# santurini/vsrlab

Measured on AMD Instinct MI355X. Metric: LR frames/sec fwd+bwd, BasicVSR 4x 540p 7-frame clip, 1->8 MI355X, higher is better.
Workload: dtype bf16; 1 GPU; BasicVSR(mid=64,res_blocks=30,x4) fwd+Charbonnier+bwd+clip+Adam, 540x960->2160x3840, 7-frame clip, 2 clips per GPU (BASELINE configs[1]); clips_per_gpu=2, frames=7, res_blocks=30, parallelism=single GPU, arena=full, train_flow=False, trunk_chains=True

## Files before the change

vsrlab_amd/csrc/conv3x3_c64_tile.h:

```cpp
#pragma once
#include "common.h"

constexpr int PTW = 32, PTH = 8, PNT = 512;
constexpr int PTWH = PTW + 2, PTHH = PTH + 2, PNPIX = PTHH * PTWH;
constexpr int W_BYTES = 9 * 64 * 64 * 2;
constexpr int IN_BYTES = PNPIX * 128;
constexpr int BIAS_OFF = W_BYTES + 2 * IN_BYTES;
constexpr int IN_CHUNKS = PNPIX * 8;
constexpr int NPIECE_T = (IN_CHUNKS + 63) / 64;
constexpr int NPIECE_W = (NPIECE_T + 3) / 4;
constexpr int WCH = 9 * 64 * 8 / 256;

typedef __attribute__((ext_vector_type(2))) __bf16 bf16x2_t;
typedef __attribute__((ext_vector_type(4))) unsigned u32x4_t;
typedef __attribute__((ext_vector_type(2))) unsigned u32x2_t;
#define GP(T, x) ((__attribute__((address_space(1))) T*)(x))

static __device__ __forceinline__ unsigned pk_bf16(float a, float b) {
    bf16x2_t p = {(bf16_t)a, (bf16_t)b};
    return __builtin_bit_cast(unsigned, p);
}
static __device__ __forceinline__ unsigned pk_max_i16(unsigned a, unsigned b) { unsigned r; asm("v_pk_max_i16 %0, %1, %2" : "=v"(r) : "v"(a), "v"(b)); return r; }
static __device__ __forceinline__ unsigned pk_min_u16(unsigned a, unsigned b) { unsigned r; asm("v_pk_min_u16 %0, %1, %2" : "=v"(r) : "v"(a), "v"(b)); return r; }
static __device__ __forceinline__ unsigned pk_mul_lo_u16(unsigned a, unsigned b) { unsigned r; asm("v_pk_mul_lo_u16 %0, %1, %2" : "=v"(r) : "v"(a), "v"(b)); return r; }
// ... 54 lines not shown
#define C64_RES_IDENTITY(idA, l15, q)                                                                                    \
    bf16x8_t idA[2];                                                                                                     \
    _Pragma("unroll") for (int hb = 0; hb < 2; ++hb)                                                                     \
        _Pragma("unroll") for (int j = 0; j < 8; ++j) idA[hb][j] = (bf16_t)(((q) == ((l15) >> 2) && j == 4 * hb + ((l15) & 3)) ? 1.f : 0.f);
#define C64_ADD_RESIDUAL(acc, idA, rr)                                                                                 \
    _Pragma("unroll") for (int nb = 0; nb < 4; ++nb)                                                                   \
        _Pragma("unroll") for (int mb = 0; mb < 4; ++mb)                                                               \
            acc[mb][nb] = __builtin_amdgcn_mfma_f32_16x16x32_bf16(idA[mb & 1], __builtin_bit_cast(bf16x8_t, rr[mb >> 1][nb]), acc[mb][nb], 0, 0, 0);

#define C64_DSR(dst, addr, imm) asm volatile("ds_read_b128 %0, %1 offset:%2" : "=v"(dst) : "v"(addr), "i"(imm))
#define C64_LOADA(tap_, kk_, slot, mb)                                                                                 \
    C64_DSR(fa_[slot][mb], (tap_ < 6 ? a_lo[kk_] : a_hi[kk_]), (tap_ < 6 ? tap_ : tap_ - 6) * 8192 + (mb) * 2048);
#define C64_LOADB(ky_, kx_, kk_, slot, nb)                                                                             \
    C64_DSR(fb_[slot][nb], bb_, (((nb) >> 1) + ky_) * (PTWH * 128) + kk_ * (4 * PTWH * 16) + (((nb) & 1) * 16 + kx_) * 16);
#define C64_LOAD(s, slot)                                                                                              \
    {                                                                                                                  \
        constexpr int tap_ = (s) / 2, kk_ = (s) % 2, ky_ = tap_ / 3, kx_ = tap_ % 3;                                   \
        C64_LOADA(tap_, kk_, slot, 0) C64_LOADA(tap_, kk_, slot, 1) C64_LOADA(tap_, kk_, slot, 2) C64_LOADA(tap_, kk_, slot, 3) \
        C64_LOADB(ky_, kx_, kk_, slot, 0) C64_LOADB(ky_, kx_, kk_, slot, 1) C64_LOADB(ky_, kx_, kk_, slot, 2) C64_LOADB(ky_, kx_, kk_, slot, 3) \
    }
#define C64_MFMA(acc, bvec, s, mb, nb) acc[mb][nb] = __builtin_amdgcn_mfma_f32_16x16x32_bf16(fa_[(s) % 2][mb], fb_[(s) % 2][nb], (s) == 0 ? bvec[mb] : acc[mb][nb], 0, 0, 0);
#define C64_ML_A(acc, bvec, s, mb, nb, lmb)                                                                            \
    C64_MFMA(acc, bvec, s, mb, nb)                                                                                     \
    __builtin_amdgcn_sched_barrier(0);                       \
    if ((s) + 1 < 18) { constexpr int t1_ = ((s) + 1) / 2, k1_ = ((s) + 1) % 2; C64_LOADA(t1_, k1_, ((s) + 1) % 2, lmb) } \
    __builtin_amdgcn_sched_barrier(0);
#define C64_ML_B(acc, bvec, s, mb, nb, lnb)                                                                            \
    C64_MFMA(acc, bvec, s, mb, nb)                                                                                     \
    __builtin_amdgcn_sched_barrier(0);                                                                                 \
    if ((s) + 1 < 18) { constexpr int t1_ = ((s) + 1) / 2, k1_ = ((s) + 1) % 2; C64_LOADB(t1_ / 3, t1_ % 3, k1_, ((s) + 1) % 2, lnb) } \
    __builtin_amdgcn_sched_barrier(0);
#define C64_STEP(acc, bvec, s)                                                                                         \
    {                                                                                                                  \
        asm volatile("s_waitcnt lgkmcnt(0)" ::: "memory");                                 \
        __builtin_amdgcn_sched_barrier(0);                                                                             \
        C64_ML_A(acc, bvec, s, 0, 0, 0) C64_ML_A(acc, bvec, s, 0, 1, 1) C64_ML_A(acc, bvec, s, 0, 2, 2) C64_ML_A(acc, bvec, s, 0, 3, 3) \
        C64_ML_B(acc, bvec, s, 1, 0, 0) C64_ML_B(acc, bvec, s, 1, 1, 1) C64_ML_B(acc, bvec, s, 1, 2, 2) C64_ML_B(acc, bvec, s, 1, 3, 3) \
        C64_MFMA(acc, bvec, s, 2, 0) C64_MFMA(acc, bvec, s, 2, 1) C64_MFMA(acc, bvec, s, 2, 2) C64_MFMA(acc, bvec, s, 2, 3)  \
        C64_MFMA(acc, bvec, s, 3, 0) C64_MFMA(acc, bvec, s, 3, 1) C64_MFMA(acc, bvec, s, 3, 2) C64_MFMA(acc, bvec, s, 3, 3)  \
        __builtin_amdgcn_sched_barrier(0);                                                                             \
    }
#define C64_K_LOOP(acc, bvec, cur)                                                                                                    \
    {                                                                                                                  \
        bf16x8_t fa_[2][4], fb_[2][4];                                                                                 \
        const unsigned bb_ = (unsigned)(W_BYTES + (cur) * IN_BYTES + (b_lane));      \
        asm volatile("s_waitcnt lgkmcnt(0)" ::: "memory");                         \
        __builtin_amdgcn_sched_barrier(0);                                                                             \
        C64_LOAD(0, 0)                                                                                                 \
        C64_STEP(acc, bvec, 0) C64_STEP(acc, bvec, 1) C64_STEP(acc, bvec, 2) C64_STEP(acc, bvec, 3) C64_STEP(acc, bvec, 4) C64_STEP(acc, bvec, 5) \
        C64_STEP(acc, bvec, 6) C64_STEP(acc, bvec, 7) C64_STEP(acc, bvec, 8) C64_STEP(acc, bvec, 9) C64_STEP(acc, bvec, 10) C64_STEP(acc, bvec, 11) \
        C64_STEP(acc, bvec, 12) C64_STEP(acc, bvec, 13) C64_STEP(acc, bvec, 14) C64_STEP(acc, bvec, 15) C64_STEP(acc, bvec, 16) C64_STEP(acc, bvec, 17) \
    }

constexpr unsigned C64_K11 = 0x00010001u;
#define C64_ARM_PLAIN(ow, v)                                                                                             \
    _Pragma("unroll") for (int jj = 0; jj < 4; ++jj) ow[jj] = pk_bf16(v[2 * jj], v[2 * jj + 1]);
#define C64_ARM_RELU(ow, v, nb, sign_k)                                                                                  \
    _Pragma("unroll") for (int jj = 0; jj < 4; ++jj) {                                                                   \
        ow[jj] = pk_max_i16(pk_bf16(v[2 * jj], v[2 * jj + 1]), 0u);                                                      \
        sign_k |= pk_min_u16(ow[jj], C64_K11) << (4 * (nb) + jj);                                                        \
    }
#define C64_ARM_MASKED(ow, v, nb, wbits)                                                                                 \
    _Pragma("unroll") for (int jj = 0; jj < 4; ++jj)                                                                     \
        ow[jj] = pk_mul_lo_u16(pk_bf16(v[2 * jj], v[2 * jj + 1]), ((wbits) >> (4 * (nb) + jj)) & C64_K11);
static __device__ __forceinline__ long long c64_sign_word(int tile, int w4, int lane) { return (long long)tile * 256 + w4 * 64 + lane; }
```

vsrlab_amd/csrc/conv3x3_persist.hip:

```cpp
#include "conv3x3_c64_tile.h"
#include <type_traits>

namespace {

constexpr int P_LDS = BIAS_OFF + 256;

__device__ uint4 g_conv_zero_chunk[2];

template <int ACT> __device__ __forceinline__ float p_act(float v, float slope) {
    if (ACT == ACT_RELU) return v > 0.f ? v : 0.f;
    if (ACT == ACT_LEAKY) return v > 0.f ? v : slope * v;
    return v;
}

#ifdef VSR_CLOCK
__device__ unsigned long long g_clk[256 * 4];
#endif

__device__ __forceinline__ void tile_coords(int tile, int ntx, int nty, int& n, int& ty0, int& tx0) {
    const int per = ntx * nty;
    n = tile / per;
    const int r = tile - n * per;
    const int ty = r / ntx;
    ty0 = ty * PTH;
    tx0 = (r - ty * ntx) * PTW;
}

struct TileIter {
    int tile, n, ty, tx;
    int sn, sty, stx;
    __device__ __forceinline__ void init(int first, int stride, int ntx, int nty) {
        const int per = ntx * nty;
        tile = first; n = first / per; int r = first - n * per; ty = r / ntx; tx = r - ty * ntx;
        sn = stride / per; r = stride - sn * per; sty = r / ntx; stx = r - sty * ntx;
    }
    __device__ __forceinline__ void advance(int stride, int ntx, int nty) {
        tile += stride;
        tx += stx; if (tx >= ntx) { tx -= ntx; ++ty; }
        ty += sty; if (ty >= nty) { ty -= nty; ++n; }
        n += sn;
    }
};

__device__ __forceinline__ float bf_lo(unsigned w) { return __uint_as_float(w << 16); }
__device__ __forceinline__ float bf_hi(unsigned w) { return __uint_as_float(w & 0xffff0000u); }

constexpr int DMA_PLAIN = 0;

template <int ACT, bool HAS_RES, int MASK>
__global__ __launch_bounds__(PNT, 1) void conv3x3_c64_persist_kernel(const ConvArgs ka) {
    extern __shared__ __attribute__((aligned(16))) char smem[];

    const int z = blockIdx.y;
// ... 165 lines not shown
                                }
                            }
                            C64_ARM_PLAIN(ow, v)
                        }
                        const u32x4_t o = {ow[0], ow[1], ow[2], ow[3]};
                        *GP(u32x4_t, dst + k * 1024) = o;
                    }
                }
            }
            };
            if (full) epilogue(std::true_type{}); else epilogue(std::false_type{});
            if (ACT != ACT_NONE && !HAS_RES && sout_z) sout_z[c64_sign_word(tile, w4, lane)] = u32x2_t{sout[0], sout[1]};
            __syncthreads();
            cur ^= 1;
        }
    }
#ifdef VSR_CLOCK
    if (tid == 0 && blockIdx.y == 0 && blockIdx.x < 256) {
        g_clk[blockIdx.x * 4 + 0] = __builtin_amdgcn_s_memtime() - clk_t0;
        g_clk[blockIdx.x * 4 + 1] = __builtin_amdgcn_s_memrealtime() - clk_r0;
    }
#endif
}

__global__ void sign_bits_c64_kernel(const bf16_t* __restrict__ x, uint2* __restrict__ bits, int N, int H, int W) {
    const int ntx = cdiv(W, PTW), nty = cdiv(H, PTH);
    const long long total = (long long)N * ntx * nty * 256;
    const long long gid = (long long)blockIdx.x * blockDim.x + threadIdx.x;
    if (gid >= total) return;
    const int lane = (int)(gid & 63), w4 = (int)((gid >> 6) & 3);
    const int tile = (int)(gid >> 8);
    const int l15 = lane & 15, q = lane >> 4;
    const int pxl = PM_LANE_PIXEL(l15);
    int n, ty0, tx0;
    tile_coords(tile, ntx, nty, n, ty0, tx0);
    unsigned out[2] = {0u, 0u};
#pragma unroll
    for (int nb = 0; nb < 4; ++nb) {
        const int yy = ty0 + 2 * w4 + (nb >> 1), xx = tx0 + (nb & 1) * 16 + pxl;
        if (yy < H && xx < W) {
#pragma unroll
            for (int k = 0; k < 2; ++k) {
                const uint4 v = *reinterpret_cast<const uint4*>(x + (long long)n * pm_image_elems(H, W, 64) + pm_off(yy, xx, 4 * k + q, W, 64));
                const unsigned vw[4] = {v.x, v.y, v.z, v.w};
#pragma unroll
                for (int jj = 0; jj < 4; ++jj)
                    out[k] |= ((bf_lo(vw[jj]) > 0.f ? 1u : 0u) | (bf_hi(vw[jj]) > 0.f ? 0x10000u : 0u)) << (4 * nb + jj);
            }
        }
    }
    bits[gid] = make_uint2(out[0], out[1]);
}

template <int ACT, bool HAS_RES, int MASK>
static int launch_persist(const ConvArgs& a, int num_cus, hipStream_t st) {
    auto kern = conv3x3_c64_persist_kernel<ACT, HAS_RES, MASK>;
    static VsrDevOnce once;
    { const int rc = vsr_set_max_dynamic_lds(once, reinterpret_cast<const void*>(kern), P_LDS); if (rc != VSR_OK) return rc; }
    const int tiles = a.N * cdiv(a.W, PTW) * cdiv(a.H, PTH);
    int gx = num_cus / a.nz;
    gx &= ~7;
    if (gx < 8) gx = num_cus / a.nz;
    if (gx < 1) gx = 1;
    if (gx > tiles) gx = tiles;
    hipLaunchKernelGGL(kern, dim3(gx, a.nz), dim3(PNT), P_LDS, st, a);
    HIP_CHECK_RET(hipGetLastError());
    return VSR_OK;
}

}

#ifdef VSR_CLOCK
extern "C" int vsr_debug_read_clk(unsigned long long* host_out) {
    return hipMemcpyFromSymbol(host_out, HIP_SYMBOL(g_clk), sizeof(unsigned long long) * 256 * 4) == hipSuccess ? 0 : -3;
}
#endif

int vsr_launch_conv3x3_c64_persist(const ConvArgs& a, int num_cus, hipStream_t st) {
    bool res = false, aux = false;
    for (int z = 0; z < a.nz; ++z) { res = res || a.res[z]; aux = aux || a.aux[z]; }
    for (int z = 0; z < a.nz; ++z) if ((res && !a.res[z]) || (aux && !a.aux[z])) return VSR_ERR_UNSUPPORTED;
    int mask = aux ? a.mask_mode : MASK_NONE;
    if (mask == MASK_RELU && !res) {
        bool bits = true;
        for (int z = 0; z < a.nz; ++z) bits = bits && a.sign_bits[z];
        if (bits) mask = MASK_RELU_BITS;
    }
    if (mask == MASK_LEAKY && res) {
        bool bits = true;
        for (int z = 0; z < a.nz; ++z) bits = bits && a.sign_bits[z];
        if (bits) mask = MASK_LEAKY_BITS;
    }
    if (pm_image_elems((PTHH + 2) * a.in_step, a.Ws, 64) * 2 > 0x7fffffffLL || pm_image_elems(2 * PTH + 2, a.Wd, 64) > 0x7fffffffLL)
        return VSR_ERR_UNSUPPORTED;
    if (a.unshuffle) {
        if (a.nz != 1 || a.out_step != 1 || a.out_ox[0] || a.out_oy[0] || (a.Hd & 1) || (a.Wd & 1) || a.Hd != a.H || a.Wd != a.W || aux ||
            a.unshuffle_plane < (long long)a.N * pm_image_elems(a.Hd / 2, a.Wd / 2, 64) || a.dst_nstride != pm_image_elems(a.Hd / 2, a.Wd / 2, 64) ||
            3 * a.unshuffle_plane + pm_image_elems(PTH + 2, a.Wd / 2, 64) > 0x7fffffffLL)
            return VSR_ERR_UNSUPPORTED;
    }
#define PERSIST_CASE(ACT, RES, MASK) if (a.act == ACT && res == RES && mask == MASK) return launch_persist<ACT, RES, MASK>(a, num_cus, st);
    PERSIST_CASE(ACT_RELU, false, MASK_NONE)
    PERSIST_CASE(ACT_NONE, true, MASK_NONE)
    PERSIST_CASE(ACT_LEAKY, false, MASK_NONE)
    PERSIST_CASE(ACT_NONE, false, MASK_NONE)
    PERSIST_CASE(ACT_NONE, false, MASK_RELU)
    PERSIST_CASE(ACT_NONE, false, MASK_RELU_BITS)
    PERSIST_CASE(ACT_NONE, true, MASK_LEAKY)
    PERSIST_CASE(ACT_NONE, true, MASK_LEAKY_BITS)
    PERSIST_CASE(ACT_NONE, false, MASK_LEAKY)
#undef PERSIST_CASE
    return VSR_ERR_UNSUPPORTED;
}

int vsr_launch_sign_bits_c64(const void* x_pm, void* bits, int N, int H, int W, hipStream_t st) {
    if (!x_pm || !bits || N < 1 || H < 1 || W < 1) return VSR_ERR_BADARG;
    const long long total = (long long)N * cdiv(W, PTW) * cdiv(H, PTH) * 256;
    hipLaunchKernelGGL(sign_bits_c64_kernel, dim3((unsigned)((total + 255) / 256)), dim3(256), 0, st, (const bf16_t*)x_pm, (uint2*)bits, N, H, W);
    HIP_CHECK_RET(hipGetLastError());
    return VSR_OK;
}
```

vsrlab_amd/csrc/kernels.h:

```cpp
#pragma once
#include "common.h"

int vsr_launch_conv(int dtype, int ks, int nsrc, int ca, int cb, int last_planar, int cout_t, int epi,
                    const ConvArgs& a, hipStream_t st);
int vsr_launch_sign_bits_c64(const void* x_pm, void* bits, int N, int H, int W, hipStream_t st);

enum { CHAIN_RELU = 0,
       CHAIN_SKIP = 1,
       CHAIN_MASK = 2 };
#define VSR_CHAIN_MAX_LAYERS 64
struct ChainLayer { unsigned src, dst, res, sbits, sout, w, bias; int variant; };
struct ChainArgs {
    char* base;
    unsigned* sync;
    int N, H, W, nlayers;
    ChainLayer layer[VSR_CHAIN_MAX_LAYERS];
};
size_t vsr_chain_sync_bytes(int nlayers, int N, int H, int W);
int vsr_launch_conv3x3_chain(const ChainArgs& a, int num_cus, hipStream_t st);
void vsr_wgrad_slab_dims(int ks, int cx, int cout, int* coutp, int* cxp, int* stride);
int vsr_launch_wgrad(int dtype, int ks, int cx, int x_planar, int cout, int dy_planar, const WgradArgs& a, int nwg,
                     int* nslabs, hipStream_t st);
int vsr_launch_wgrad_reduce(const float* slab, int nwg, int ks, int cx, int cout, int cout_real, int cin_real, float* gw,
                            int I_total, int i_off, int o_mul, int o_add, float* gb, int accumulate, hipStream_t st);
int vsr_launch_warp_fwd(int dtype, const void* in, const float* flow, void* out, int N, int H, int W, int C,
                        long long flow_nstride, hipStream_t st, int border = 0);
int vsr_launch_warp_bwd(int dtype, const void* dout, const float* flow, float* dacc, int N, int H, int W, int C,
                        long long flow_nstride, hipStream_t st, int border = 0);
int vsr_launch_warp_bwd_gather(int dtype, const void* dout, const float* flow, const void* dtop, long long* S, int* far_count, void* out,
                               int N, int H, int W, int C, long long flow_nstride, hipStream_t st);
int vsr_launch_add_cast(int dtype, const void* a, const float* s, void* out, int N, int H, int W, int C, hipStream_t st);
int vsr_launch_planar_to_pm(int dtype, const float* in, void* out, int N, int Cin, int H, int W, int C, hipStream_t st);
int vsr_launch_pm_to_planar(int dtype, const void* in, float* out, int N, int Cout, int H, int W, int C, hipStream_t st);
int vsr_launch_resize_norm(const float* in, float* out, const float* mean, const float* std, int F, int h, int w, int hu,
                           int wu, hipStream_t st);
int vsr_launch_avgpool2(const float* in, float* out, long long planes, int h, int w, hipStream_t st);
int vsr_launch_spynet_prepare(int dtype, const float* frames, const float* flow_prev, float* flow_up, void* x16, int n,
                              int t, int P, int pair_mode, int h, int w, int level0, hipStream_t st);
int vsr_launch_flow_out(const float* in, float* out, int P, int hu, int wu, int h, int w, hipStream_t st);
int vsr_launch_warp_bwd_flow(int dtype, const void* in, const void* dout, const float* flow, float* dflow, int N, int H, int W,
                             int C, long long flow_nstride, hipStream_t st, int border = 0);
int vsr_launch_spynet_dres(int dtype, const float* dflow, const float* res, void* out, int P, int h, int w, hipStream_t st);
int vsr_launch_spynet_prepare_bwd(int dtype, const void* dx16, const float* dflow_l, const float* frames, const float* flow_up,
                                  float* dflow_prev, float* dframes, int n, int t, int P, int pair_mode, int h, int w, hipStream_t st);
int vsr_launch_avgpool2_bwd_add(const float* dcoarse, float* dfine, long long planes, int h, int w, hipStream_t st);
int vsr_launch_resize_norm_bwd(const float* dnorm, float* dframes, const float* std, int F, int h, int w, int hu, int wu, hipStream_t st);
int vsr_launch_bilinear4_bwd(const float* dsr, float* dlr, long long planes, int h, int w, hipStream_t st, int scale = 4);
int vsr_launch_flow_out_bwd(const float* dout, float* din, int P, int hu, int wu, int h, int w, hipStream_t st);
int vsr_launch_add_f32(const float* a, const float* b, float* out, long long n, hipStream_t st);
int vsr_launch_c64_to_planar(const ConvArgs& a, hipStream_t st);
int vsr_launch_last2_wgrad(const void* x, const float* dy, long long dy_nstride, float* slab, int slab_stride, int N, int H, int W,
                           int* nslabs, hipStream_t st, int pc = 3);
int vsr_launch_last2_dgrad(const float* dsr, long long dsr_nstride, const float* w, const void* aux, void* dst, int N, int H, int W,
                           int mask_mode, hipStream_t st, const void* sign_bits = nullptr, float slope = 0.f);
struct VsrPackDesc {
    const float* w; void* dst;
    int total, blk0;
// ... 35 lines not shown
```

vsrlab_amd/csrc/layer_ops.hip:

```cpp
#include "recipes.h"

constexpr int C64 = 64;

extern "C" {

static bool layer_width_ok(int c) { return c == 16 || c == 32 || c == 64; }

int vsr_flow_warp_fwd(int dtype, const void* in_pm, const float* flow, void* out_pm, int N, int H, int W, int Cc, void* stream) {
    return vsr_flow_warp_fwd_ex(dtype, in_pm, flow, out_pm, N, H, W, Cc, 0, stream);
}
int vsr_flow_warp_bwd(int dtype, const void* dout_pm, const float* flow, float* dacc, int N, int H, int W, int Cc, void* stream) {
    return vsr_flow_warp_bwd_ex(dtype, dout_pm, flow, dacc, N, H, W, Cc, 0, stream);
}
int vsr_flow_warp_bwd_flow(int dtype, const void* in_pm, const void* dout_pm, const float* flow, float* dflow, int N, int H, int W,
                           int Cc, void* stream) {
    return vsr_flow_warp_bwd_flow_ex(dtype, in_pm, dout_pm, flow, dflow, N, H, W, Cc, 0, stream);
}
int vsr_flow_warp_fwd_ex(int dtype, const void* in_pm, const float* flow, void* out_pm, int N, int H, int W, int Cc, int padding_mode,
                         void* stream) {
    if (bad_dtype(dtype) || !in_pm || !flow || !out_pm || bad_dims(N, H, W) || Cc < 16 || (Cc & 15) || (padding_mode & ~1)) return VSR_ERR_BADARG;
    return vsr_launch_warp_fwd(dtype, in_pm, flow, out_pm, N, H, W, Cc, (long long)2 * H * W, (hipStream_t)stream, padding_mode);
}
int vsr_flow_warp_bwd_ex(int dtype, const void* dout_pm, const float* flow, float* dacc, int N, int H, int W, int Cc, int padding_mode,
                         void* stream) {
// ... 121 lines not shown
        }
        if (dlr_planar) {
            CK(c.pack_stem_dlr(w, wp, cat));
            CK(c.conv_planar3(dyM, wp, nullptr, dlr_planar, (long long)3 * H * W, nullptr, N, H, W));
        }
        if (gw) {
            WgradArgs a = wg_base(N, H, W, C, C), af = a;
            a.x[0] = lr_planar; a.x_nstride = (long long)3 * H * W; a.dy[0] = dyM;
            af.x[0] = x_pm; af.dy[0] = dyM;
            CK(c.stem_wgrads(cat, a, af, gw, gb, 0));
        }
        return VSR_OK;
    }
    if (ks == 3 || ks == 1) {
        const int C = cin_pm;
        if (!layer_width_ok(C) || cin_real != C || !x_pm) return VSR_ERR_UNSUPPORTED;
        const Ctx c(nullptr, st, dtype, C, slab);
        if (pixel_shuffle) {
            if (ks != 3 || cout_real != 4 * C || cd != C || act != ACT_NONE) return VSR_ERR_UNSUPPORTED;
            if (dx_pm) {
                CK(c.pack_ps(w, wp, 1));
                CK(c.conv_ps_dgrad(dyM, wp, dx_pm, nullptr, 0, N, H, W));
            }
            if (gw) CK(c.ps_wgrads(&x_pm, &dyM, 1, false, N, H, W, gw, gb, 0));
            return VSR_OK;
        }
        if (cout_real != C || cd != C) return VSR_ERR_UNSUPPORTED;
        if (dx_pm) {
            CK(c.pack_cc(ks, w, wp, 1));
            CK(c.conv(ks, dyM, wp, nullptr, dx_pm, ACT_NONE, nullptr, nullptr, 0, N, H, W));
        }
        if (gw) {
            WgradArgs a = wg_base(N, H, W, C, C);
            a.x[0] = x_pm; a.dy[0] = dyM;
            CK(c.wgrad_cc(ks, a, gw, C, 0, gb, 0));
        }
        return VSR_OK;
    }
    if (ks != 7 || pixel_shuffle || !x_pm) return VSR_ERR_UNSUPPORTED;
    for (int j = 0; j < NSPY; ++j) {
        if (cin_pm != SPY_CIP[j] || cout_real != SPY_CO[j] || cin_real != SPY_CI[j]) continue;
        if (j < NSPY - 1 && cd != SPY_CD[j]) return VSR_ERR_BADARG;
        const Ctx c(nullptr, st, dtype, 64, slab);
        if (gw) CK(c.spy_wgrad(j, x_pm, dyM, N, H, W, gw, gb, 0));
        if (dx_pm) {
            CK(c.pack_spy(j, w, wp, 1));
            CK(c.spy_dgrad(j, dyM, wp, dx_pm, nullptr, N, H, W));
        }
        return VSR_OK;
    }
    return VSR_ERR_UNSUPPORTED;
}

int vsr_conv_layer_fwd(int dtype, int ks, const void* x_pm, int cin_pm, const float* lr_planar, const float* w, const float* b,
                       int cin_real, int cout_real, void* wpack, void* y_pm, int cd, float* y_planar, int act, float slope,
                       int pixel_shuffle, int N, int H, int W, void* stream) {
    if (bad_dtype(dtype) || !w || !wpack || bad_dims(N, H, W) || (!x_pm && !lr_planar) || (!y_pm && !y_planar) || act < ACT_NONE || act > ACT_LEAKY)
        return VSR_ERR_BADARG;
    hipStream_t st = (hipStream_t)stream;
    char* wp = (char*)wpack;
    if (lr_planar) {
        const int C = cout_real;
        if (ks != 3 || !layer_width_ok(C) || !y_pm || cd != C || pixel_shuffle) return VSR_ERR_UNSUPPORTED;
        const bool cat = x_pm != nullptr;
        if (cat ? (cin_pm != C || cin_real != C + 3) : cin_real != 3) return VSR_ERR_UNSUPPORTED;
        const Ctx c(nullptr, st, dtype, C);
        CK(c.pack_stem(w, wp, cat));
        return c.stem(cat, x_pm, lr_planar, (long long)3 * H * W, wp, b, y_pm, act, slope, N, H, W);
    }
    if (ks == 3 || ks == 1) {
        const int C = cin_pm;
        if (!layer_width_ok(C) || cin_real != C) return VSR_ERR_UNSUPPORTED;
        const Ctx c(nullptr, st, dtype, C);
        if (pixel_shuffle) {
            if (ks != 3 || cout_real != 4 * C || !y_pm || cd != C) return VSR_ERR_UNSUPPORTED;
            CK(c.pack_ps(w, wp, 0));
            float* b4 = reinterpret_cast<float*>(wp + (size_t)4 * 9 * c.CO * C * c.es);
            if (b) CK(c.pack_ps_bias(b, b4));
            return c.conv_ps(x_pm, wp, b ? b4 : nullptr, y_pm, N, H, W, act, slope);
        }
        if (cout_real != C || !y_pm || cd != C) return VSR_ERR_UNSUPPORTED;
        CK(c.pack_cc(ks, w, wp, 0));
        return c.conv(ks, x_pm, wp, b, y_pm, act, nullptr, nullptr, 0, N, H, W, nullptr, nullptr, false, slope);
    }
    if (ks != 7 || pixel_shuffle) return VSR_ERR_UNSUPPORTED;
    for (int j = 0; j < NSPY; ++j) {
        if (cin_pm != SPY_CIP[j] || cout_real != SPY_CO[j] || cin_real != SPY_CI[j]) continue;
        const Ctx c(nullptr, st, dtype);
        CK(c.pack_spy(j, w, wp, 0));
        if (j < NSPY - 1 ? (!y_pm || cd != SPY_CD[j]) : !y_planar) return VSR_ERR_BADARG;
        return c.spy_conv(j, x_pm, wp, b, j < NSPY - 1 ? y_pm : (void*)y_planar, act, slope, nullptr, N, H, W);
    }
    return VSR_ERR_UNSUPPORTED;
}

size_t vsr_conv3x3_c64_wgrad_slab_floats(void) { return wgrad_slab_floats(); }

int vsr_conv3x3_c64_wgrad(int dtype, const void* x_pm, const void* dy_pm, float* gw, float* gb, float* slab, int N, int H, int W,
                          void* stream) {
    if (bad_dtype(dtype) || !x_pm || !dy_pm || !gw || !slab || bad_dims(N, H, W)) return VSR_ERR_BADARG;
    const Ctx c(nullptr, (hipStream_t)stream, dtype, 64, slab);
    WgradArgs a = wg_base(N, H, W);
    a.x[0] = x_pm; a.dy[0] = dy_pm;
    return c.wgrad(a, {3, 64, false, 64, false}, {C64, C64, gw, C64, 0, 1, 0, gb, 0}, false);
}

// ... 8 lines not shown
```

vsrlab_amd/csrc/recipes.h:

```cpp
#pragma once
#include <vector>
#include "host.h"

inline constexpr int NSPY = 5;
inline constexpr int SPY_CI[NSPY] = {8, 32, 64, 32, 16};
inline constexpr int SPY_CO[NSPY] = {32, 64, 32, 16, 2};
inline constexpr int SPY_CIP[NSPY] = {16, 32, 64, 32, 16};
inline constexpr int SPY_COP[NSPY] = {32, 64, 32, 32, 32};
inline constexpr int SPY_CD[NSPY] = {32, 64, 32, 16, 0};
inline constexpr int SPY_DK[NSPY] = {32, 64, 32, 16, 16};
inline constexpr int SPY_DROWS[NSPY] = {32, 32, 64, 32, 32};

struct Ctx {
    char* ws;
    hipStream_t st;
    int dtype;
    int C, CO;
    size_t es;
    float* slab;
    mutable std::vector<VsrPackDesc>* batch = nullptr;
    Ctx(char* ws_, hipStream_t st_, int dtype_, int C_ = 64, float* slab_ = nullptr)
        : ws(ws_), st(st_), dtype(dtype_), C(C_), CO(C_ < 32 ? 32 : C_), es(esize(dtype_)), slab(slab_) {}
    void* at(size_t off) const { return ws + off; }
    const float* fat(size_t off) const { return reinterpret_cast<const float*>(ws + off); }

    static long long plane_elems(int N, int H, int W) { return (long long)N * pm_image_elems(H / 2, W / 2, 64); }
    static void set_unshuffle(ConvArgs& a, int N, int H, int W) {
        a.unshuffle = 1; a.unshuffle_plane = plane_elems(N, H, W); a.dst_nstride = pm_image_elems(H / 2, W / 2, 64);
    }
    int conv(int ks, const void* x, const void* wpack, const float* bias, void* y, int act, const void* res, const void* aux, int mask,
             int N, int H, int W, void* sign_out = nullptr, const void* sign_bits = nullptr, bool unshuffle = false, float slope = 0.f) const {
        ConvArgs a = conv_args(N, H, W, C);
        a.src[0] = x; a.wpack = wpack; a.bias = bias; a.dst[0] = y; a.act = act; a.leaky_slope = slope; a.res[0] = res; a.aux[0] = aux; a.mask_mode = mask;
        a.sign_out[0] = sign_out; a.sign_bits[0] = sign_bits;
        if (unshuffle) set_unshuffle(a, N, H, W);
        const int rc = vsr_launch_conv(dtype, ks, 1, C, C, 0, CO, EPI_NHWC, a, st);
        if (rc == VSR_OK && sign_out && dtype == VSR_BF16 && vsr_env().generic_conv) return vsr_launch_sign_bits_c64(y, sign_out, N, H, W, st);
        return rc;
    }
    int conv_planar3(const void* x, const void* wpack, const float* bias, float* y, long long y_nstride, const float* pres, int N, int H, int W) const {
        ConvArgs a = conv_args(N, H, W, C);
        a.src[0] = x; a.wpack = wpack; a.bias = bias; a.cout_real = 3; a.dst[0] = y; a.dst_nstride = y_nstride; a.pres = pres;
        return vsr_launch_conv(dtype, 3, 1, C, C, 0, 32, EPI_PLANAR, a, st);
    }

    int pack_ps(const float* w, void* dst, int mode) const {
        for (int z = 0; z < 4; ++z) CK(pack(w, (char*)dst + (size_t)z * 9 * CO * C * es, 9, CO, C, C, C, C, 0, 4, z, mode));
        return VSR_OK;
    }
    int pack_ps_bias(const float* b, float* dst) const {
        for (int z = 0; z < 4; ++z) CK(pack_bias(b, dst + z * C, C, 4, z));
        return VSR_OK;
    }
    int conv_ps(const void* x, const void* wpack, const float* bias4, void* y, int N, int H, int W, int act = ACT_NONE, float slope = 0.f) const {
        ConvArgs a = conv_args(N, H, W, C);
        a.src[0] = x; a.wpack = wpack; a.w_zstride = 9 * CO * C; a.bias = bias4; a.bias_zstride = C; a.nz = 4; a.act = act; a.leaky_slope = slope;
        a.out_step = 2; a.Hd = 2 * H; a.Wd = 2 * W; a.dst_nstride = pm_image_elems(2 * H, 2 * W, C);
        for (int z = 0; z < 4; ++z) { a.dst[z] = y; a.out_oy[z] = z >> 1; a.out_ox[z] = z & 1; }
        return vsr_launch_conv(dtype, 3, 1, C, C, 0, CO, EPI_NHWC, a, st);
    }
    int conv_ps_dgrad(const void* dy, const void* wpackd, void* dx, const void* aux, int mask, int N, int H, int W, const void* sign_bits = nullptr,
                      bool dy_planes = false, bool dx_planes = false) const {
        if (dtype == VSR_BF16 && C == 64) {
            for (int z = 0; z < 4; ++z) {
                ConvArgs a = conv_args(N, H, W, C);
                if (dy_planes) {
                    a.src[0] = (const char*)dy + (size_t)z * plane_elems(N, 2 * H, 2 * W) * es;
                } else {
                    a.in_step = 2; a.Hs = 2 * H; a.Ws = 2 * W;
                    a.src[0] = dy; a.src_oy[0] = z >> 1; a.src_ox[0] = z & 1; a.src_nstride[0] = pm_image_elems(2 * H, 2 * W, C);
                }
                a.wpack = (const char*)wpackd + (size_t)z * 9 * C * C * es; a.dst[0] = dx;
                a.res[0] = z > 0 ? dx : nullptr;
                if (dx_planes) set_unshuffle(a, N, H, W);
                if (z == 3) { a.aux[0] = aux; a.mask_mode = mask; a.sign_bits[0] = aux ? sign_bits : nullptr; }
                int rc = vsr_launch_conv(dtype, 3, 1, 64, 64, 0, 64, EPI_NHWC, a, st);
                if (rc != VSR_OK) return rc;
            }
            return VSR_OK;
        }
        ConvArgs a = conv_args(N, H, W, C);
        a.nz = 1; a.in_step = 2; a.Hs = 2 * H; a.Ws = 2 * W;
        for (int s = 0; s < 4; ++s) { a.src[s] = dy; a.src_oy[s] = s >> 1; a.src_ox[s] = s & 1; a.src_nstride[s] = pm_image_elems(2 * H, 2 * W, C); }
        a.wpack = wpackd; a.dst[0] = dx; a.aux[0] = aux; a.mask_mode = mask;
        return vsr_launch_conv(dtype, 3, 4, C, C, 0, CO, EPI_NHWC, a, st);
    }
    int ps_wgrads(const void* const* x, const void* const* dy, int nseg, bool dy_planes, int N, int H, int W, float* gw, float* gb, int accumulate) const {
        for (int z = 0; z < 4; ++z) {
            WgradArgs a = wg_base(N, H, W, C, C);
            a.nseg = nseg;
            for (int i = 0; i < nseg; ++i) {
                a.x[i] = x[i];
                a.dy[i] = dy_planes ? (const char*)dy[i] + (size_t)z * plane_elems(N, 2 * H, 2 * W) * es : dy[i];
            }
            if (!dy_planes) { a.dy_step = 2; a.dy_oy = z >> 1; a.dy_ox = z & 1; a.Hy = 2 * H; a.Wy = 2 * W; a.dy_nstride = pm_image_elems(2 * H, 2 * W, C); }
            CK(wgrad(a, {3, C, false, C, false}, {C, C, gw, C, 0, 4, z, gb, accumulate}));
        }
        return VSR_OK;
    }

    int pack_stem(const float* w, void* dst, bool cat) const {
        const int I_total = cat ? C + 3 : 3;
        if (cat) CK(pack(w, dst, 9, CO, C, C, C, I_total, 3, 1, 0, 0));
        return pack(w, (char*)dst + (cat ? (size_t)9 * CO * C * es : 0), 9, CO, 16, C, 3, I_total, 0, 1, 0, 0);
    }
    int pack_stem_dgrad(const float* w, void* dst) const { return pack(w, dst, 9, CO, C, C, C, C + 3, 3, 1, 0, 1); }
    int pack_stem_dlr(const float* w, void* dst, bool cat) const { return pack(w, dst, 9, 32, C, 3, C, cat ? C + 3 : 3, 0, 1, 0, 1); }
    int stem(bool cat, const void* feat, const float* lr, long long lr_nstride, const void* wpack, const float* bias, void* y, int act, float slope,
             int N, int H, int W) const {
        ConvArgs a = conv_args(N, H, W, C);
        a.wpack = wpack; a.bias = bias; a.dst[0] = y; a.act = act; a.leaky_slope = slope;
        a.src[cat ? 1 : 0] = lr; a.src_nstride[cat ? 1 : 0] = lr_nstride;
        if (!cat) return vsr_launch_conv(dtype, 3, 1, 16, 16, 1, CO, EPI_NHWC, a, st);
        a.src[0] = feat;
        return vsr_launch_conv(dtype, 3, 2, C, 16, 1, CO, EPI_NHWC, a, st);
    }
// ... 67 lines not shown
```

Before: 58.51 LR frames/s.

## Fuse four pixel-shuffle dgrad phase convs into one persistent kernel

Adds a persistent 64-channel 3x3 kernel for the pixel-shuffle data gradient. It accumulates all four sub-pixel phases in registers, so the output tile is written once instead of being read back and re-added across four separate launches. A DMA role of waves streams each phase's weights and input tile into LDS with double buffering, while the compute waves run MFMA over the four K-loops. It is used only when dy arrives as phase planes and the generic path is off, and it falls back to the old path when the arguments are unsupported.

```diff
diff --git a/vsrlab_amd/csrc/conv3x3_c64_tile.h b/vsrlab_amd/csrc/conv3x3_c64_tile.h
--- a/vsrlab_amd/csrc/conv3x3_c64_tile.h
+++ b/vsrlab_amd/csrc/conv3x3_c64_tile.h
@@ -130,6 +130,39 @@
         C64_STEP(acc, bvec, 12) C64_STEP(acc, bvec, 13) C64_STEP(acc, bvec, 14) C64_STEP(acc, bvec, 15) C64_STEP(acc, bvec, 16) C64_STEP(acc, bvec, 17) \
     }
 
+#define C64_MFMA_ACC0(acc, mb, nb) acc[mb][nb] = __builtin_amdgcn_mfma_f32_16x16x32_bf16(fa_[0][mb], fb_[0][nb], acc[mb][nb], 0, 0, 0);
+#define C64_ML_A_ACC0(acc, mb, nb, lmb)                                                                                \
+    C64_MFMA_ACC0(acc, mb, nb)                                                                                         \
+    __builtin_amdgcn_sched_barrier(0);                                                                                 \
+    C64_LOADA(0, 1, 1, lmb)                                                \
+    __builtin_amdgcn_sched_barrier(0);
+#define C64_ML_B_ACC0(acc, mb, nb, lnb)                                                                                \
+    C64_MFMA_ACC0(acc, mb, nb)                                                                                         \
+    __builtin_amdgcn_sched_barrier(0);                                                                                 \
+    C64_LOADB(0, 0, 1, 1, lnb)                                                                                         \
+    __builtin_amdgcn_sched_barrier(0);
+#define C64_STEP0_ACC(acc)                                                                                             \
+    {                                                                                                                  \
+        asm volatile("s_waitcnt lgkmcnt(0)" ::: "memory");                                                             \
+        __builtin_amdgcn_sched_barrier(0);                                                                             \
+        C64_ML_A_ACC0(acc, 0, 0, 0) C64_ML_A_ACC0(acc, 0, 1, 1) C64_ML_A_ACC0(acc, 0, 2, 2) C64_ML_A_ACC0(acc, 0, 3, 3)  \
+        C64_ML_B_ACC0(acc, 1, 0, 0) C64_ML_B_ACC0(acc, 1, 1, 1) C64_ML_B_ACC0(acc, 1, 2, 2) C64_ML_B_ACC0(acc, 1, 3, 3)  \
+        C64_MFMA_ACC0(acc, 2, 0) C64_MFMA_ACC0(acc, 2, 1) C64_MFMA_ACC0(acc, 2, 2) C64_MFMA_ACC0(acc, 2, 3)            \
+        C64_MFMA_ACC0(acc, 3, 0) C64_MFMA_ACC0(acc, 3, 1) C64_MFMA_ACC0(acc, 3, 2) C64_MFMA_ACC0(acc, 3, 3)            \
+        __builtin_amdgcn_sched_barrier(0);                                                                             \
+    }
+#define C64_K_LOOP_ACC(acc, bvec, cur)                                                                                 \
+    {                                                                                                                  \
+        bf16x8_t fa_[2][4], fb_[2][4];                                                                                 \
+        const unsigned bb_ = (unsigned)(W_BYTES + (cur) * IN_BYTES + (b_lane));                                        \
+        asm volatile("s_waitcnt lgkmcnt(0)" ::: "memory");                                                             \
+        __builtin_amdgcn_sched_barrier(0);                                                                             \
+        C64_LOAD(0, 0)                                                                                                 \
+        C64_STEP0_ACC(acc) C64_STEP(acc, bvec, 1) C64_STEP(acc, bvec, 2) C64_STEP(acc, bvec, 3) C64_STEP(acc, bvec, 4) C64_STEP(acc, bvec, 5) \
+        C64_STEP(acc, bvec, 6) C64_STEP(acc, bvec, 7) C64_STEP(acc, bvec, 8) C64_STEP(acc, bvec, 9) C64_STEP(acc, bvec, 10) C64_STEP(acc, bvec, 11) \
+        C64_STEP(acc, bvec, 12) C64_STEP(acc, bvec, 13) C64_STEP(acc, bvec, 14) C64_STEP(acc, bvec, 15) C64_STEP(acc, bvec, 16) C64_STEP(acc, bvec, 17) \
+    }
+
 constexpr unsigned C64_K11 = 0x00010001u;
 #define C64_ARM_PLAIN(ow, v)                                                                                             \
     _Pragma("unroll") for (int jj = 0; jj < 4; ++jj) ow[jj] = pk_bf16(v[2 * jj], v[2 * jj + 1]);
diff --git a/vsrlab_amd/csrc/conv3x3_persist.hip b/vsrlab_amd/csrc/conv3x3_persist.hip
--- a/vsrlab_amd/csrc/conv3x3_persist.hip
+++ b/vsrlab_amd/csrc/conv3x3_persist.hip
@@ -1,4 +1,5 @@
 #include "conv3x3_c64_tile.h"
+#include "ps_dgrad_args.h"
 #include <type_traits>
 
 namespace {
@@ -270,6 +271,205 @@
     bits[gid] = make_uint2(out[0], out[1]);
 }
 
+template <int MASK>
+__global__ __launch_bounds__(PNT, 1) void conv3x3_c64_psd_kernel(const ConvArgs ka) {
+    extern __shared__ __attribute__((aligned(16))) char smem[];
+    struct {
+        int N, H, W, unshuffle;
+        long long src_nstride0, dst_nstride, plane;
+        unsigned long long src0, src1, wpack, aux, sign_bits, dst; float leaky_slope;
+    } a = {ka.N, ka.H, ka.W, ka.unshuffle, ka.src_nstride[0], ka.dst_nstride, ka.unshuffle_plane,
+           (unsigned long long)ka.src[0], (unsigned long long)ka.src[1], (unsigned long long)ka.wpack, (unsigned long long)ka.aux[0],
+           (unsigned long long)ka.sign_bits[0], (unsigned long long)ka.dst[0], ka.leaky_slope};
+    asm volatile("" : "+s"(a.N), "+s"(a.H), "+s"(a.W), "+s"(a.unshuffle), "+s"(a.src_nstride0), "+s"(a.dst_nstride), "+s"(a.plane));
+    asm volatile("" : "+s"(a.src0), "+s"(a.src1), "+s"(a.wpack), "+s"(a.aux), "+s"(a.sign_bits), "+s"(a.dst), "+s"(a.leaky_slope));
+    const int tid = threadIdx.x, lane = tid & 63, wave = tid >> 6;
+    const int role = __builtin_amdgcn_readfirstlane(wave >> 2);
+    const int w4 = wave & 3;
+    const int l15 = lane & 15, q = lane >> 4;
+    const int pxl = PM_LANE_PIXEL(l15);
+    char* lds_w = smem;
+    char* lds_t = smem + W_BYTES;
+#ifdef VSR_CLOCK
+    unsigned long long clk_t0 = 0, clk_r0 = 0, clk_ab = 0, clk_items = 0;
+    if (tid == 0) { clk_t0 = __builtin_amdgcn_s_memtime(); clk_r0 = __builtin_amdgcn_s_memrealtime(); }
+#endif
+
+    const int ntx = cdiv(a.W, PTW), nty = cdiv(a.H, PTH);
+    const int WS = pm_ws(a.W);
+    const TileWalk walk = xcd_tile_walk(a.N * ntx * nty, blockIdx.x, gridDim.x);
+    if (walk.first >= walk.end) return;
+    const unsigned long long pstep = a.src1 - a.src0;
+
+    if (role == 1) {
+        const auto* zsrc = GP(const char, g_conv_zero_chunk);
+        int rel[NPIECE_W];
+        C64_DMA_REL(rel, w4, lane, 1, 0, 0, WS)
+        u32x4_t wvp[WCH];
+        const int pt = tid & 255;
+        auto issue = [&](const TileIter& it, long long plane_off, int buf) {
+            const int n = it.n, ty0 = it.ty * PTH, tx0 = it.tx * PTW;
+            const auto* org = GP(const char, a.src0 + (unsigned long long)plane_off) + ((long long)n * a.src_nstride0 + pm_off(ty0, tx0, 0, a.W, 64)) * 2;
+            char* dstb = lds_t + buf * IN_BYTES;
+            C64_DMA_TILE(DMA_PLAIN, rel, org, zsrc, dstb, w4, lane, ty0, tx0, a.H, a.W)
+        };
+        TileIter it;
+        it.init(walk.first, walk.stride, ntx, nty);
+        issue(it, 0ll, 0);
+        asm volatile("s_waitcnt vmcnt(0)" ::: "memory");
+        __syncthreads();
+        int j = 1, buf = 0, tile_j, z;
+        long long woff, poff;
+        psd_item(j, walk.first, walk.stride, (long long)pstep, &tile_j, &z, &woff, &poff);
+        {
+            const auto* wgz = GP(const u32x4_t, a.wpack + (unsigned long long)woff);
+            C64_W_LOAD(wvp, wgz, pt)
+        }
+        issue(it, poff, 1);
+        for (;;) {
+            asm volatile("s_waitcnt vmcnt(0)" ::: "memory");
+            __syncthreads();
+            const bool more = it.tile < walk.end;
+            if (more) { C64_W_STORE(wvp, lds_w, pt) }
+            __syncthreads();
+            if (!more) break;
+            psd_item(++j, walk.first, walk.stride, (long long)pstep, &tile_j, &z, &woff, &poff);
+            if (z == 0) it.advance(walk.stride, ntx, nty);
+            if (it.tile < walk.end) {
+                const auto* wgz = GP(const u32x4_t, a.wpack + (unsigned long long)woff);
+                C64_W_LOAD(wvp, wgz, pt)
+                issue(it, poff, buf);
+            }
+            buf ^= 1;
+        }
+    } else {
+        u32x4_t wv[WCH];
+        {
+            const auto* wg0 = GP(const u32x4_t, a.wpack);
+            C64_W_LOAD(wv, wg0, tid)
+        }
+        C64_MFMA_LANE(w4, l15, q, pxl)
+        int loff[4];
+#pragma unroll
+        for (int nb = 0; nb < 4; ++nb) {
+            const int row = w4 * 2 + (nb >> 1), px = (nb & 1) * 16 + pxl;
+            loff[nb] = ((row * WS) * 8 + q) * 256 + px * 8;
+            if (a.unshuffle) loff[nb] = (int)(((row & 1) * 2 + (px & 1)) * a.plane) + (((row >> 1) * pm_ws(a.W >> 1)) * 8 + q) * 256 + (px >> 1) * 8;
+        }
+        C64_W_STORE(wv, lds_w, tid)
+        asm volatile("s_waitcnt vmcnt(0)" ::: "memory");
+        __syncthreads();
+        auto* const dst_z = GP(bf16_t, a.dst);
+        const auto* const aux_z = GP(const bf16_t, a.aux);
+        const auto* const sbits_z = GP(const u32x2_t, a.sign_bits);
+        const float slope = vsr_slope(a.leaky_slope);
+        f32x4_t bvec[4];
+#pragma unroll
+        for (int mb = 0; mb < 4; ++mb) bvec[mb] = f32x4_t{0.f, 0.f, 0.f, 0.f};
+        constexpr bool BITS = MASK == MASK_LEAKY_BITS;
+        static_assert(MASK == MASK_NONE || MASK == MASK_LEAKY || MASK == MASK_LEAKY_BITS, "the masks a pixel-shuffle data gradient is launched with");
+
+#ifdef VSR_CLOCK
+#define PSD_CLK_A unsigned long long clk_a_ = 0; if (tid == 0) clk_a_ = __builtin_amdgcn_s_memtime();
+#define PSD_CLK_B if (tid == 0) { clk_ab += __builtin_amdgcn_s_memtime() - clk_a_; ++clk_items; }
+#else
+#define PSD_CLK_A
+#define PSD_CLK_B
+#endif
+        int cur = 0;
+        TileIter it;
+        for (it.init(walk.first, walk.stride, ntx, nty); it.tile < walk.end; it.advance(walk.stride, ntx, nty)) {
+            const int tile = it.tile, n = it.n, ty0 = it.ty * PTH, tx0 = it.tx * PTW;
+            const long long tbase = a.unshuffle ? (long long)n * a.dst_nstride + pm_off(ty0 >> 1, tx0 >> 1, 0, a.W >> 1, 64)
+                                                : (long long)n * a.dst_nstride + pm_off(ty0, tx0, 0, a.W, 64);
+            const bool full = ty0 + PTH <= a.H && tx0 + PTW <= a.W;
+            bool ok[4];
+#pragma unroll
+            for (int nb = 0; nb < 4; ++nb) ok[nb] = (tx0 + (nb & 1) * 16 + pxl < a.W) && (ty0 + w4 * 2 + (nb >> 1) < a.H);
+
+            f32x4_t acc[4][4];
+            {
+                C64_K_LOOP(acc, bvec, cur)
+                PSD_CLK_A
+                __syncthreads();
+                __syncthreads();
+                PSD_CLK_B
+                cur ^= 1;
+            }
+#pragma unroll 1
+            for (int z = 1; z < 3; ++z) {
+                C64_K_LOOP_ACC(acc, bvec, cur)
+                PSD_CLK_A
+                __syncthreads();
+                __syncthreads();
+                PSD_CLK_B
+                cur ^= 1;
+            }
+            u32x4_t mm[2][4];
+            u32x2_t sbits = {0u, 0u};
+            if (BITS) sbits = sbits_z[c64_sign_word(tile, w4, lane)];
+            if (MASK == MASK_LEAKY) {
+#pragma unroll
+                for (int nb = 0; nb < 4; ++nb) {
+                    if (full || ok[nb]) {
+#pragma unroll
+                        for (int k = 0; k < 2; ++k) mm[k][nb] = *GP(const u32x4_t, aux_z + tbase + loff[nb] + k * 1024);
+                    }
+                }
+            }
+            C64_K_LOOP_ACC(acc, bvec, cur)
+            PSD_CLK_A
+            __syncthreads();
+            if (MASK != MASK_NONE) __builtin_amdgcn_s_waitcnt(0x0F70);
+            auto epilogue = [&](auto FULL) {
+#pragma unroll
+                for (int nb = 0; nb < 4; ++nb) {
+                    if (decltype(FULL)::value || ok[nb]) {
+                        auto* dst = dst_z + tbase + loff[nb];
+#pragma unroll
+                        for (int k = 0; k < 2; ++k) {
+                            float v[8];
+#pragma unroll
+                            for (int j = 0; j < 4; ++j) { v[j] = acc[2 * k][nb][j]; v[4 + j] = acc[2 * k + 1][nb][j]; }
+                            if (BITS) {
+                                const unsigned wbits = k ? sbits.y : sbits.x;
+#pragma unroll
+                                for (int j = 0; j < 8; ++j) v[j] *= ((wbits >> (4 * nb + (j >> 1) + 16 * (j & 1))) & 1u) ? 1.f : slope;
+                            } else if (MASK == MASK_LEAKY) {
+                                const u32x4_t mq = mm[k][nb];
+                                const unsigned mw[4] = {mq.x, mq.y, mq.z, mq.w};
+#pragma unroll
+                                for (int jj = 0; jj < 4; ++jj) {
+                                    v[2 * jj] *= (bf_lo(mw[jj]) > 0.f ? 1.f : slope);
+                                    v[2 * jj + 1] *= (bf_hi(mw[jj]) > 0.f ? 1.f : slope);
+                                }
+                            }
+                            unsigned ow[4];
+                            C64_ARM_PLAIN(ow, v)
+                            const u32x4_t o = {ow[0], ow[1], ow[2], ow[3]};
+                            *GP(u32x4_t, dst + k * 1024) = o;
+                        }
+                    }
+                }
+            };
+            if (full) epilogue(std::true_type{}); else epilogue(std::false_type{});
+            __syncthreads();
+            PSD_CLK_B
+            cur ^= 1;
+        }
+#undef PSD_CLK_A
+#undef PSD_CLK_B
+    }
+#ifdef VSR_CLOCK
+    if (tid == 0 && blockIdx.x < 256) {
+        g_clk[blockIdx.x * 4 + 0] = __builtin_amdgcn_s_memtime() - clk_t0;
+        g_clk[blockIdx.x * 4 + 1] = __builtin_amdgcn_s_memrealtime() - clk_r0;
+        g_clk[blockIdx.x * 4 + 2] = clk_ab;
+        g_clk[blockIdx.x * 4 + 3] = clk_items;
+    }
+#endif
+}
+
 template <int ACT, bool HAS_RES, int MASK>
 static int launch_persist(const ConvArgs& a, int num_cus, hipStream_t st) {
     auto kern = conv3x3_c64_persist_kernel<ACT, HAS_RES, MASK>;
@@ -331,6 +531,23 @@
     return VSR_ERR_UNSUPPORTED;
 }
 
+int vsr_launch_conv3x3_c64_ps_dgrad(const ConvArgs& a, int num_cus, hipStream_t st) {
+    const int mask = psd_check(a);
+    if (mask < 0) return mask;
+    auto kern = mask == MASK_LEAKY_BITS ? conv3x3_c64_psd_kernel<MASK_LEAKY_BITS>
+              : mask == MASK_LEAKY ? conv3x3_c64_psd_kernel<MASK_LEAKY> : conv3x3_c64_psd_kernel<MASK_NONE>;
+    static VsrDevOnce once[3];
+    { const int rc = vsr_set_max_dynamic_lds(once[mask == MASK_LEAKY_BITS ? 2 : mask == MASK_LEAKY ? 1 : 0], reinterpret_cast<const void*>(kern), P_LDS); if (rc != VSR_OK) return rc; }
+    const int tiles = a.N * cdiv(a.W, PTW) * cdiv(a.H, PTH);
+    int gx = num_cus & ~7;
+    if (gx < 8) gx = num_cus;
+    if (gx < 1) gx = 1;
+    if (gx > tiles) gx = tiles;
+    hipLaunchKernelGGL(kern, dim3(gx), dim3(PNT), P_LDS, st, a);
+    HIP_CHECK_RET(hipGetLastError());
+    return VSR_OK;
+}
+
 int vsr_launch_sign_bits_c64(const void* x_pm, void* bits, int N, int H, int W, hipStream_t st) {
     if (!x_pm || !bits || N < 1 || H < 1 || W < 1) return VSR_ERR_BADARG;
     const long long total = (long long)N * cdiv(W, PTW) * cdiv(H, PTH) * 256;
diff --git a/vsrlab_amd/csrc/kernels.h b/vsrlab_amd/csrc/kernels.h
--- a/vsrlab_amd/csrc/kernels.h
+++ b/vsrlab_amd/csrc/kernels.h
@@ -3,6 +3,7 @@
 
 int vsr_launch_conv(int dtype, int ks, int nsrc, int ca, int cb, int last_planar, int cout_t, int epi,
                     const ConvArgs& a, hipStream_t st);
+int vsr_launch_conv3x3_c64_ps_dgrad(const ConvArgs& a, int num_cus, hipStream_t st);
 int vsr_launch_sign_bits_c64(const void* x_pm, void* bits, int N, int H, int W, hipStream_t st);
 
 enum { CHAIN_RELU = 0,
diff --git a/vsrlab_amd/csrc/layer_ops.hip b/vsrlab_amd/csrc/layer_ops.hip
--- a/vsrlab_amd/csrc/layer_ops.hip
+++ b/vsrlab_amd/csrc/layer_ops.hip
@@ -197,6 +197,15 @@
     return VSR_ERR_UNSUPPORTED;
 }
 
+extern "C" int vsr_debug_conv_ps_dgrad(const void* dy_pm, const float* w, void* wpack, void* dx_pm, const void* aux_pm, void* sign_bits,
+                                       int dy_planes, int dx_planes, int N, int H, int W, void* stream) {
+    if (!dy_pm || !w || !wpack || !dx_pm || bad_dims(N, H, W) || (sign_bits && !aux_pm)) return VSR_ERR_BADARG;
+    const Ctx c(nullptr, (hipStream_t)stream, VSR_BF16);
+    CK(c.pack_ps(w, wpack, 1));
+    if (sign_bits) CK(vsr_launch_sign_bits_c64(aux_pm, sign_bits, N, H, W, (hipStream_t)stream));
+    return c.conv_ps_dgrad(dy_pm, wpack, dx_pm, aux_pm, aux_pm ? MASK_LEAKY : MASK_NONE, N, H, W, sign_bits, dy_planes != 0, dx_planes != 0);
+}
+
 int vsr_conv_layer_fwd(int dtype, int ks, const void* x_pm, int cin_pm, const float* lr_planar, const float* w, const float* b,
                        int cin_real, int cout_real, void* wpack, void* y_pm, int cd, float* y_planar, int act, float slope,
                        int pixel_shuffle, int N, int H, int W, void* stream) {
diff --git a/vsrlab_amd/csrc/ps_dgrad_args.h b/vsrlab_amd/csrc/ps_dgrad_args.h
--- /dev/null
+++ b/vsrlab_amd/csrc/ps_dgrad_args.h
@@ -0,0 +1,50 @@
+#pragma once
+#include "host.h"
+
+constexpr int PSD_PHASES = 4;
+constexpr long long PSD_WSET_ELEMS = 9 * 64 * 64;
+
+inline long long psd_plane_elems(int N, int H, int W) { return (long long)N * pm_image_elems(H, W, 64); }
+inline ConvArgs psd_args(const void* dy, const void* wpackd, void* dx, const void* aux, int mask, const void* sign_bits, bool dx_planes,
+                         int N, int H, int W) {
+    ConvArgs a = conv_args(N, H, W, 64);
+    for (int z = 0; z < PSD_PHASES; ++z) a.src[z] = (const char*)dy + (size_t)z * psd_plane_elems(N, H, W) * 2;
+    a.wpack = wpackd; a.w_zstride = PSD_WSET_ELEMS; a.dst[0] = dx;
+    a.aux[0] = aux; a.mask_mode = aux ? mask : MASK_NONE; a.sign_bits[0] = aux ? sign_bits : nullptr;
+    if (dx_planes) { a.unshuffle = 1; a.unshuffle_plane = (long long)N * pm_image_elems(H / 2, W / 2, 64); a.dst_nstride = pm_image_elems(H / 2, W / 2, 64); }
+    return a;
+}
+
+inline int psd_check(const ConvArgs& a) {
+    if (a.N < 1 || a.H < 1 || a.W < 1 || !a.wpack || !a.dst[0]) return VSR_ERR_BADARG;
+    for (int z = 0; z < PSD_PHASES; ++z) if (!a.src[z]) return VSR_ERR_BADARG;
+    const ptrdiff_t pstep = (const char*)a.src[1] - (const char*)a.src[0];
+    if (pstep < psd_plane_elems(a.N, a.H, a.W) * 2 || (pstep & 15)) return VSR_ERR_UNSUPPORTED;
+    for (int z = 2; z < PSD_PHASES; ++z) if ((const char*)a.src[z] - (const char*)a.src[z - 1] != pstep) return VSR_ERR_UNSUPPORTED;
+    if (a.in_step != 1 || a.out_step != 1 || a.Hs != a.H || a.Ws != a.W || a.Hd != a.H || a.Wd != a.W || a.nz != 1 || a.CD != 64 || a.cout_real != 64 ||
+        a.src_nstride[0] != pm_image_elems(a.H, a.W, 64) || a.w_zstride != PSD_WSET_ELEMS || a.bias || a.res[0] || a.act != ACT_NONE ||
+        a.out_ox[0] || a.out_oy[0] || a.sign_out[0])
+        return VSR_ERR_UNSUPPORTED;
+    int mask = MASK_NONE;
+    if (a.aux[0]) {
+        if (a.mask_mode != MASK_LEAKY) return VSR_ERR_UNSUPPORTED;
+        mask = a.sign_bits[0] ? MASK_LEAKY_BITS : MASK_LEAKY;
+    }
+    if (pm_image_elems(10 + 2, a.W, 64) * 2 > 0x7fffffffLL || pm_image_elems(2 * 8 + 2, a.W, 64) > 0x7fffffffLL) return VSR_ERR_UNSUPPORTED;
+    if (a.unshuffle) {
+        if (mask == MASK_LEAKY) return VSR_ERR_UNSUPPORTED;
+        if ((a.H & 1) || (a.W & 1) || a.unshuffle_plane < (long long)a.N * pm_image_elems(a.H / 2, a.W / 2, 64) ||
+            a.dst_nstride != pm_image_elems(a.H / 2, a.W / 2, 64) || 3 * a.unshuffle_plane + pm_image_elems(8 + 2, a.W / 2, 64) > 0x7fffffffLL)
+            return VSR_ERR_UNSUPPORTED;
+    } else if (a.dst_nstride != pm_image_elems(a.H, a.W, 64)) {
+        return VSR_ERR_UNSUPPORTED;
+    }
+    return mask;
+}
+
+static inline __host__ __device__ void psd_item(int j, int first, int stride, long long plane_bytes, int* tile, int* z, long long* wset_off, long long* plane_off) {
+    *tile = first + (j >> 2) * stride;
+    *z = j & 3;
+    *wset_off = (long long)*z * PSD_WSET_ELEMS * 2;
+    *plane_off = (long long)*z * plane_bytes;
+}
diff --git a/vsrlab_amd/csrc/recipes.h b/vsrlab_amd/csrc/recipes.h
--- a/vsrlab_amd/csrc/recipes.h
+++ b/vsrlab_amd/csrc/recipes.h
@@ -1,6 +1,7 @@
 #pragma once
 #include <vector>
 #include "host.h"
+#include "ps_dgrad_args.h"
 
 inline constexpr int NSPY = 5;
 inline constexpr int SPY_CI[NSPY] = {8, 32, 64, 32, 16};
@@ -62,6 +63,10 @@
     int conv_ps_dgrad(const void* dy, const void* wpackd, void* dx, const void* aux, int mask, int N, int H, int W, const void* sign_bits = nullptr,
                       bool dy_planes = false, bool dx_planes = false) const {
         if (dtype == VSR_BF16 && C == 64) {
+            if (dy_planes && !vsr_env().generic_conv) {
+                const int rc = vsr_launch_conv3x3_c64_ps_dgrad(psd_args(dy, wpackd, dx, aux, mask, sign_bits, dx_planes, N, H, W), vsr_num_cus(), st);
+                if (rc != VSR_ERR_UNSUPPORTED) return rc;
+            }
             for (int z = 0; z < 4; ++z) {
                 ConvArgs a = conv_args(N, H, W, C);
                 if (dy_planes) {
```

Result: no change. 59.01 LR frames/s, median of 6 (+0.9%).
